# Complexity-ML/complexity-tokenizer

Hardware: AMD Instinct MI355X
Metric: MB/s raw UTF-8 encoded (encode_batch), 50k ByteLevel BPE, 1/2/4/8 MI355X (higher is better)
Workload: dtype u8

## Files before the change

complexity-tokenizer_amd/csrc/ctok_encode.cpp:

```cpp
#include <chrono>
#include <cstdio>
#include <cstring>

#include "call_plan.h"
#include "gen/unicode_data.h"
#include "host_internal.h"
#include "knobs.h"

ctok::ctok() = default;
ctok::~ctok() = default;

namespace ctok_rt __attribute__((visibility("hidden"))) {

bool cp_fast_ok() {
  static const bool ok = [] {
    if (process_knobs().no_cp_ranges) return false;
    for (uint32_t cp = 0x3000; cp < 0x1F700; cp++) {
      const int rc = cp_range_class(cp);
      if (rc < 0) continue;
      const int cl = (ct_cls_stage2[ct_cls_stage1[cp >> 8] * 64 + ((cp & 255) >> 2)] >> ((cp & 3) * 2)) & 3;
      if (cl != rc || ct_nfc_stage2[ct_nfc_stage1[cp >> 8] * 256 + (cp & 255)] != 0) return false;
    }
    return true;
  }();
// ... 331 lines not shown
  Capacities cap{};
  Work w{};
  bool tm = false;
  PassPlan plan{};
  Laps laps;
  uint64_t ntok = 0;
  uint32_t cnt[kNumCounters] = {};
};

void normalise(Enc& e, Attempt& a) {
  ctok* t = e.t;
  DeviceState* ds = e.ds;
  const EncodeCall& c = e.c;
  hipStream_t s = c.stream;
  const uint64_t n_docs = c.n_docs;
  const bool nfc = t->nfc && c.n_bytes;
  a.ev0_marker = c.timing && (t->add_prefix_space || (nfc && (c.all_nfc || !a.speculate)));
  if (a.ev0_marker) HIPTRY(hipEventRecord(ds->ev[kEvStart], s));
  ds->counters.ensure(kCounterWords);
  a.text = c.text, a.off = c.doc_off, a.B = c.n_bytes;
  a.norm = t->add_prefix_space;
  if (nfc && c.all_nfc) {
    ds->doc_flag.ensure(n_docs + 1);
    HIPTRY(hipMemsetD32Async((hipDeviceptr_t)ds->doc_flag.p, 1, n_docs + 1, s));
    a.nfc_docs = n_docs;
    a.norm = true;
  } else if (nfc && !a.speculate) {
    ds->doc_flag.ensure(n_docs + 1);
    HIPTRY(hipMemsetAsync(ds->doc_flag.p, 0, (n_docs + 1) * 4, s));
    HIPTRY(hipMemsetAsync(ds->counters.p, 0, kCounterWords * 4, s));
    a.ctr_zeroed = true;
    STEP("nfc_check", launch_nfc_check(c.text, c.n_bytes, c.doc_off, (uint32_t)n_docs, e.tb, ds->doc_flag.p,
                                       ds->counters.p + kCtrNfcDocs, s));
    HIPTRY(hipMemcpyAsync(ds->host + kPinScratch, ds->counters.p + kCtrNfcDocs, 4, hipMemcpyDeviceToHost, s));
    spin_sync(ds, s);
    a.nfc_docs = *pinned<uint32_t>(ds, kPinScratch);
    if (a.nfc_docs) a.norm = true;
  }
  if (a.norm) {
    const int do_nfc = t->nfc && a.nfc_docs;
    ds->doc_flag.ensure(n_docs + 1);
    if (!t->nfc) HIPTRY(hipMemsetAsync(ds->doc_flag.p, 0, (n_docs + 1) * 4, s));
    ds->ncp.ensure(n_docs + 1);
    ds->norm_off.ensure(n_docs + 2);
    ds->cps.ensure(4 * c.n_bytes + 64);
    STEP("norm0", launch_norm(c.text, c.doc_off, (uint32_t)n_docs, ds->doc_flag.p, t->add_prefix_space, do_nfc, e.tb,
                              ds->cps.p, ds->ncp.p, ds->norm_off.p, nullptr, 0, s));
    ds->scan_tmp.ensure(scan_tmp_elems(n_docs + 1) + 64);
    HIPTRY(scan_u64(ds->norm_off.p, n_docs, ds->scan_tmp.p, ds->scan_tmp.cap, s));
    HIPTRY(hipMemcpyAsync(ds->host + kPinScratch, ds->norm_off.p + n_docs, 8, hipMemcpyDeviceToHost, s));
    spin_sync(ds, s);
    const uint64_t nb = *pinned<uint64_t>(ds, kPinScratch);
    if (nb >= 0xF0000000ull) throw_err(CTOK_E_ARG, "normalised batch exceeds 3.75 GiB; split the batch");
    ds->norm_text.ensure(nb + 16);
    STEP("norm1", launch_norm(c.text, c.doc_off, (uint32_t)n_docs, ds->doc_flag.p, t->add_prefix_space, do_nfc, e.tb,
                              ds->cps.p, ds->ncp.p, ds->norm_off.p, ds->norm_text.p, 1, s));
    a.text = ds->norm_text.p, a.off = ds->norm_off.p, a.B = nb;
  }
  if (a.B > 0 && ((uintptr_t)a.text & 15)) throw_err(CTOK_E_ARG, "device text buffer must be 16-byte aligned");
  ds->last_norm = a.norm;
  ds->last_B = a.B;
}

template <class T, class P>
void bind(DevBuf<T>& b, size_t n, P*& field) {
  b.ensure(n);
  field = (P*)b.p;
}

void size_workspace(Enc& e, Attempt& a) {
  DeviceState* ds = e.ds;
  const ProcessKnobs& pk = process_knobs();
  Work& w = a.w;
  w.text = a.text;
  w.n_bytes = (uint32_t)a.B;
  w.doc_off = a.off;
  w.n_docs = (uint32_t)e.c.n_docs;
  w.n_words = (uint32_t)((a.B + 31) / 32);
  w.n_tiles = (uint32_t)((a.B + kTile - 1) / kTile);
  w.n_cus = ds->n_cus;
  w.nfc_watch = a.speculate ? (e.splice ? 2u : 1u) : 0u;
  w.keep_first = e.c.mode == EncodeMode::KeepFirst ? 1u : 0u;
  w.short_wgs = e.knobs.short_wgs;
  const size_t nt = w.n_tiles;
  a.cap = plan_capacities(a.B, nt, a.safe, e.tb.n_at, pk.unit, e.knobs.c3_sparse);
  w.k0 = a.cap.k0;
  w.unit = a.cap.unit;
  w.long_cap = a.cap.long_cap;
  w.mid_cap = a.cap.mid_cap;
  w.c3_max = a.cap.c3_max;
  w.rec16 = (e.t->narrow && !pk.rec32) ? 1u : 0u;
  ds->last_rec16 = (int)w.rec16;

  if (w.nfc_watch == 2) bind(ds->nfc_bits, nfc_bits_words(a.B), w.nfc_bits);
  bind(ds->tfirst, nt + 8, w.tfirst);
  bind(ds->pbits, w.n_words + 8, w.pbits);
  bind(ds->wpref, nt * 64 + 8, w.wpref);
  bind(ds->tile_np, nt + 8, w.tile_np);
  bind(ds->tile_tok, nt + 8, w.tile_tok);
  bind(ds->tile_doc, nt + 8, w.tile_doc);
  bind(ds->tcls, kNumClasses * nt + 8, w.tcls);
  bind(ds->list0, nt * w.k0 + 8, w.list0);
  bind(ds->rend, kNumClasses * nt + 8, w.rend);
  if (e.tb.n_at == 0) {
    ds->list1.ensure(nt * kCap1 + 8);
    ds->list2.ensure(nt * kCap2 + 8);
    ds->list3.ensure(nt * kCap3 + 8);
  }
  w.list1 = ds->list1.p, w.list2 = ds->list2.p, w.list3 = ds->list3.p;
  bind(ds->tcnt, nt * kTileSlots + 8, w.tcnt);
  bind(ds->prec, nt * kTileSlots * (w.rec16 ? 1 : 2) + 16, w.prec);
  bind(ds->mrec, nt * kTileSlots + 8, w.mrec);
  bind(ds->pdoc, nt * (kTileSlots / 32) + 8, w.pdoc);
  bind(ds->scratch, nt * kTileSlots + 8, w.scratch);
  bind(ds->tregion, nt + 8, w.tregion);
  bind(ds->long_list, w.long_cap + 8, w.long_list);
  bind(ds->long_cnt, w.long_cap + 8, w.long_cnt);
  bind(ds->long_ord, w.long_cap + 8, w.long_ord);
  bind(ds->long_hist, kLhWords, w.long_hist);
  bind(ds->mid_list, w.mid_cap + 8, w.mid_list);
  bind(ds->scan_tmp, std::max(scan_tmp_elems(std::max<uint64_t>(nt + 1, e.c.n_docs + 1)), tile_scan_tmp_elems(nt)) + 64,
       w.scan_tmp);
  w.scan_tmp_cap = ds->scan_tmp.cap * 2;
  w.counters = ds->counters.p;
  if (w.c3_max) {
    bind(ds->c3q, w.c3_max + 8, w.c3q);
    bind(ds->c3pre, kC3Shards + 8, w.c3pre);
  }
  w.report = (uint32_t*)(ds->host_dev + kPinReport);
  w.host_res = pk.copy_results ? nullptr : ds->host_dev + kPinNtok;
  hipStream_t s = e.c.stream;
#ifdef CTOK_CHECK
  HIPTRY(hipMemsetAsync(ds->mrec.p, 0xFF, (size_t)nt * kTileSlots * 4, s));
#endif
  if (pk.wgrec) {
    bind(ds->wgrec, kWgRecWords, w.wgrec);
    HIPTRY(hipMemsetAsync(ds->wgrec.p, 0, kWgRecWords * 8, s));
  }
  if (pk.stamps && nt) {
    bind(ds->stamps, nt * 8 + 8, w.stamps);
    HIPTRY(hipMemsetAsync(ds->stamps.p, 0, nt * 8 * 8, s));
  }
}
void bind_long_prep(DeviceState* ds, Work& w, uint32_t n_long) {
  bind(ds->long_pos, n_long + 8, w.long_pos);
  bind(ds->lw_pos, n_long + 8, w.lw_pos);
  ds->lwn.ensure(n_long + 8);
  ds->scan_tmp2.ensure(scan_tmp_elems(n_long + 1) + 64);
}
void bind_long_ids(DeviceState* ds, Work& w, uint32_t n_ids, uint32_t n_gmem_bytes) {
  bind(ds->lids, (uint64_t)n_ids + 64, w.lids);
  bind(ds->lw, 4 * (uint64_t)n_gmem_bytes + 64, w.lw);
}

Lx lx(const Enc& e, const Attempt& a, int start, int stop) {
  Lx x;
  if (a.tm && start >= 0) x.start = e.ds->ev[start];
  if (a.tm && stop >= 0) x.stop = e.ds->ev[stop];
  return x;
}


void launch_pretok(Enc& e, Attempt& a) {
  hipStream_t s = e.c.stream;
  a.tm = e.c.timing && e.c.stats && a.w.n_tiles;
  e.hp.mark(kHpPrep);
// ... 194 lines not shown
```

complexity-tokenizer_amd/csrc/ctok_internal.h:

```cpp
#pragma once
#include <hip/hip_runtime.h>

#include <cstdint>

namespace ctok_dev {

constexpr uint64_t kEmpty = ~0ull;
constexpr uint32_t kIdBits = 21;
constexpr uint64_t kKeyMask = (1ull << 42) - 1;
constexpr uint32_t kNoRank = 0x3FFFFFu;
constexpr uint32_t kMaxId = (1u << kIdBits) - 2;
constexpr uint32_t kPanicVal = kNoRank - 1;

constexpr uint32_t kErrPanic = 1u;

constexpr int kTileWords = 62;
constexpr int kTile = kTileWords * 64;
constexpr int kTileSlots = 4096;
constexpr int kSegWaves = 4;
constexpr int kSegUnroll = 4;
constexpr int kShortMax = 32;
constexpr int kMedMax = 64;
constexpr uint32_t kCap0 = kTile, kCap1 = (kTile + 8) / 9, kCap2 = (kTile + 16) / 17, kCap3 = (kTile + 32) / 33;
constexpr uint32_t kCap0Lean = 1040;
// ... 74 lines not shown
}
__host__ __device__ inline uint32_t hash16_g(uint32_t a, uint32_t b) {
  return mul24(b, 0xC2B2AFu) + mul24(a ^ 0x5A5Au, 0x27D4EBu);
}

__host__ __device__ inline uint32_t piece_hash(uint32_t lo, uint32_t hi, uint32_t len) {
  uint32_t h = mul24(lo, 0x9E3779u) + mul24((lo >> 24) | (hi << 8), 0x85EBCBu) + mul24((hi >> 16) | (len << 16), 0xC2B2AFu);
  h ^= h >> 15;
  h = mul24(h, 0x27D4EBu) ^ (h >> 9);
  return h ^ (h >> 16);
}

__host__ __device__ __forceinline__ int cp_range_class(uint32_t cp) {
  if (cp - 0x4E00u < 0x5200u) return 1;
  if (cp - 0xAC00u < 0x2BA4u) return 1;
  if (cp - 0x3041u < 0x56u) return 1;
  if (cp - 0x30A1u < 0x5Au) return 1;
  if (cp - 0x1F300u < 0x350u) return 3;
  return -1;
}

struct Tables {
  const uint64_t* merge_tab;
  uint32_t merge_mask;
  const uint4* lds_image;
  const uint32_t* pair0;
  const uint4* lds16_image;
  const uint64_t* merge16;
  uint32_t merge16_mask;
  const uint4* piece_tab;
  uint32_t piece_mask;
  const uint32_t* rank_newid;
  uint32_t n_ranks;
  const int32_t* byte2id;
  const uint8_t* cls_s1;
  const uint8_t* cls_s2;
  const uint8_t* nfc_s1;
  const uint16_t* nfc_s2;
  const uint8_t* cls_bmp;
  uint32_t cp_fast;
  const uint32_t* decomp_cp;
  const uint16_t* decomp_off;
  const uint32_t* decomp_data;
  uint32_t n_decomp;
  const uint64_t* comp_key;
  const uint32_t* comp_val;
  uint32_t n_comp;
  const uint8_t* bytemap_alnum;
  const uint8_t* at_bytes;
  const uint32_t* at_off;
  const uint32_t* at_id;
  const uint8_t* at_flags;
  uint32_t n_at;
  uint32_t proper;
  const uint32_t* eager;
  uint32_t window;
  const uint32_t* wmeta;
  uint32_t compact;
  uint32_t narrow;
  uint32_t short_packed;
  uint32_t mid_packed;
  uint32_t dbg;
  uint32_t all_bytes;
};

__host__ __device__ inline bool mid_folded(const Tables& t, uint32_t long_pieces) {
  return t.mid_packed == 2 && t.short_packed && t.n_at == 0 && long_pieces == 0;
}

struct Work {
  const uint8_t* text;
  uint32_t n_bytes;
  const uint64_t* doc_off;
  uint32_t n_docs;
  uint32_t* tfirst;
  uint32_t* pbits;
  uint32_t n_words;
  uint32_t n_tiles;
  uint32_t n_cus;
  uint32_t nfc_watch;
  uint32_t* nfc_bits;
  uint32_t mid_wide;
  uint32_t short_wgs;
  uint32_t keep_first;
  uint16_t* wpref;
  uint32_t* tile_np;
  uint32_t* tile_tok;
  uint32_t* tile_doc;
  uint32_t* tcls;
  uint32_t* list0;
  uint32_t k0;
  uint32_t* list1;
  uint32_t* list2;
  uint32_t* list3;
  void* prec;
  uint32_t rec16;
  uint32_t* mrec;
  uint32_t* pdoc;
  uint32_t* tcnt;
  uint32_t* long_cnt;
  uint32_t* long_ord;
  uint32_t* long_hist;
  uint32_t* scratch;
  uint32_t* lids;
  uint32_t* long_pos;
  uint32_t* lw_pos;
  uint32_t* rend;
  uint2* tregion;
  uint32_t long_cap, mid_cap;
  uint32_t unit;
  uint64_t* long_list;
  uint64_t* mid_list;
  uint32_t* counters;
  uint32_t* lw;
  uint32_t* scan_tmp;
  uint64_t scan_tmp_cap;
  uint64_t* stamps;
  uint32_t c3_max;
  uint32_t* c3q;
  uint32_t* c3pre;
  uint64_t* host_res;
  uint64_t* wgrec;
  uint32_t* report;
  uint32_t seq;
};

struct Lx {
  hipEvent_t start = nullptr, stop = nullptr;
};

constexpr uint32_t kDecLenMask = 0xFFFFFFu, kDecNonAscii = 1u << 30, kDecSpecial = 1u << 31;
constexpr uint32_t kDecOptSkipSpecial = 1u, kDecOptCleanup = 2u;
constexpr int kDecChunk = 4096;
constexpr int kDecTile = 4096;

struct DecTables {
  const uint2* ent;
  uint32_t n_ent;
  const uint8_t* bytes;
};

struct DecWork {
  const uint32_t* ids;
  uint32_t n_ids;
  const uint64_t* tok_off;
  uint32_t n_docs;
  uint32_t opts;
  uint32_t n_chunks;
  uint32_t* chunk_off;
  uint8_t* raw;
  uint32_t n_raw;
  uint64_t* raw_off;
  uint32_t* delbits;
  uint32_t n_tiles;
  uint32_t* tile_cnt;
  uint32_t* counters;
};

hipError_t launch_dec_len(const DecWork& w, const DecTables& t, uint32_t* tmp, uint64_t tmp_cap, hipStream_t s);
hipError_t launch_dec_gather(const DecWork& w, const DecTables& t, uint8_t* dst, uint64_t* dst_off, hipStream_t s);
hipError_t launch_dec_prepare(const DecWork& w, hipStream_t s);
hipError_t launch_dec_count(const DecWork& w, uint32_t* tmp, uint64_t tmp_cap, hipStream_t s);
hipError_t launch_dec_write(const DecWork& w, uint8_t* out, uint64_t* out_off, hipStream_t s);

constexpr uint32_t kPadItemA = 0xFFFFFFFFu;
constexpr int kPadMaxItems = 16;
// ... 79 lines not shown
```

complexity-tokenizer_amd/csrc/kernels.hip:

```cpp
#include <hip/hip_ext.h>
#include <hip/hip_runtime.h>

#include <algorithm>
#include <mutex>
#include <type_traits>

#include "ctok_internal.h"
#include "merge_packed_hd.h"
#include "seg_lane.h"

namespace ctok_dev {

#define HIPCHK(x) do { hipError_t e_ = (x); if (e_ != hipSuccess) return e_; } while (0)

template <typename F, typename... A>
static void launch_lx(const Lx& x, F k, dim3 grid, dim3 block, uint32_t lds, hipStream_t s, A... a) {
  if (x.start || x.stop)
    hipExtLaunchKernelGGL(k, grid, block, lds, s, x.start, x.stop, 0u, a...);
  else
    hipLaunchKernelGGL(k, grid, block, lds, s, a...);
}

constexpr uint32_t kNone = 0xFFFFFFFFu;
constexpr uint32_t kDead = 0xFFFFFFFFu;
constexpr uint32_t kSel = kNoRank - 1;


__device__ __forceinline__ void write_report(const Work& w) {
  const uint32_t lane = threadIdx.x & 63;
  uint32_t c3 = 0;
  if (w.c3_max) {
    const uint32_t c = w.counters[kNumCounters + lane];
    uint32_t inc = c;
#pragma unroll
    for (int o = 1; o < 64; o <<= 1) {
      const uint32_t v = (uint32_t)__shfl_up((int)inc, o, 64);
      if (lane >= (uint32_t)o) inc += v;
    }
    w.c3pre[lane] = inc - c;
    if (lane == 63) w.c3pre[64] = inc;
    c3 = __shfl((int)inc, 63, 64);
    if (__ballot(c > w.c3_max / kC3Shards)) c3 = ~0u;
  }
  if (lane < (uint32_t)kNumCounters) w.report[lane] = lane == (uint32_t)kCtrC3Count ? c3 : w.counters[lane];
  __builtin_amdgcn_fence(__ATOMIC_RELEASE, "");
  asm volatile("s_waitcnt vmcnt(0)" ::: "memory");
  if (lane == 0) __hip_atomic_store(&w.report[kNumCounters], w.seq, __ATOMIC_RELAXED, __HIP_MEMORY_SCOPE_SYSTEM);
  __builtin_amdgcn_fence(__ATOMIC_RELEASE, "");
}

__device__ __forceinline__ uint32_t wave_min_u32(uint32_t v) {
#pragma unroll
  for (int o = 32; o > 0; o >>= 1) v = min(v, (uint32_t)__shfl_xor((int)v, o, 64));
  return v;
}

__device__ __forceinline__ uint32_t wave_min_full_u32(uint32_t v) {
  v = min(v, (uint32_t)__builtin_amdgcn_update_dpp((int)v, (int)v, 0xB1, 0xF, 0xF, false));
  v = min(v, (uint32_t)__builtin_amdgcn_update_dpp((int)v, (int)v, 0x4E, 0xF, 0xF, false));
  v = min(v, (uint32_t)__builtin_amdgcn_update_dpp((int)v, (int)v, 0x141, 0xF, 0xF, false));
  v = min(v, (uint32_t)__builtin_amdgcn_update_dpp((int)v, (int)v, 0x140, 0xF, 0xF, false));
  const uint32_t a = __builtin_amdgcn_readlane(v, 0), b = __builtin_amdgcn_readlane(v, 16);
  const uint32_t c = __builtin_amdgcn_readlane(v, 32), d = __builtin_amdgcn_readlane(v, 48);
  return min(min(a, b), min(c, d));
}

__device__ __forceinline__ uint32_t wave_sum_full_u32(uint32_t v) {
  v += (uint32_t)__builtin_amdgcn_update_dpp((int)v, (int)v, 0xB1, 0xF, 0xF, false);
  v += (uint32_t)__builtin_amdgcn_update_dpp((int)v, (int)v, 0x4E, 0xF, 0xF, false);
  v += (uint32_t)__builtin_amdgcn_update_dpp((int)v, (int)v, 0x141, 0xF, 0xF, false);
  v += (uint32_t)__builtin_amdgcn_update_dpp((int)v, (int)v, 0x140, 0xF, 0xF, false);
  return __builtin_amdgcn_readlane(v, 0) + __builtin_amdgcn_readlane(v, 16) + __builtin_amdgcn_readlane(v, 32) +
         __builtin_amdgcn_readlane(v, 48);
}

__device__ __forceinline__ uint64_t lanemask_lt() {
  const uint32_t lane = threadIdx.x & 63;
  return lane ? (~0ull >> (64 - lane)) : 0ull;
}

template <typename T>
__device__ __forceinline__ T wave_incl_scan(T v) {
  const int lane = threadIdx.x & 63;
#pragma unroll
  for (int o = 1; o < 64; o <<= 1) {
    T u = __shfl_up(v, o, 64);
    if (lane >= o) v += u;
  }
  return v;
}
// ... 1090 lines not shown
    const bool has_r = q < 8;
    const uint32_t lo = lv & ((1u << bi) - 1u);
    const bool has_l = lo != 0;
    const uint32_t pv = 31u - (uint32_t)__builtin_clz(lo | 1u);
    const uint32_t L = s_tok[pv * NT + tid], R = s_tok[min(q, 7u) * NT + tid];
    s_tok[bi * NT + tid] = (uint16_t)nid;
    s_key[p * NT + tid] = ~0u;
    lv &= ~(1u << p);
    m--;
    Probe<true, HOT> pl, pr;
    pl.start(t, P, L, nid, has_l);
    pr.start(t, P, nid, R, has_r);
    const uint32_t rl = pl.finish(t, err), rr = pr.finish(t, err);
    if (has_l) s_key[pv * NT + tid] = (rl << 3) | pv;
    s_key[bi * NT + tid] = has_r ? (rr << 3) | bi : ~0u;
  }
  uint32_t* out = out_of(m);
#pragma unroll
  for (int k = 0; k < 8; k++)
    if ((lv >> k) & 1u) out[__popc(lv & ((1u << k) - 1u))] = s_tok[k * NT + tid];
  return m;
}

template <bool COMPACT, bool HOT, uint32_t NT, typename OutOf>
__device__ __forceinline__ uint32_t merge_lds8(const Tables& t, const PairLds& P, const uint32_t* tk, const uint32_t* rk,
                                               uint32_t m, lds_u32* s_key, lds_u16* s_tok, uint32_t* err,
                                               OutOf&& out_of) {
  const uint32_t tid = threadIdx.x;
#pragma unroll
  for (int k = 0; k < 8; k++) {
    s_key[k * NT + tid] = (uint32_t)k + 1 < m ? (rk[k] << 3) | (uint32_t)k : ~0u;
    s_tok[k * NT + tid] = (uint16_t)tk[k];
  }
  return merge_lds8_run<COMPACT, HOT, NT>(t, P, m, s_key, s_tok, err, out_of);
}

template <bool HOT>
struct Lookup16 {
  const Tables& t;
  const PairLds& P;
  uint32_t* err;
  Probe<true, HOT> pl, pr;
  bool has_l = false, has_r = false;
  __device__ __forceinline__ uint32_t new_id(uint32_t v) const { return v; }
  __device__ __forceinline__ void start(uint32_t L, uint32_t nid, uint32_t R, bool hl, bool hr) {
    has_l = hl;
    has_r = hr;
    pl.start(t, P, L, nid, hl);
    pr.start(t, P, nid, R, hr);
  }
  __device__ __forceinline__ void finish(uint32_t& rl, uint32_t& rr) {
    rl = (has_l ? pl.finish(t, err) : kNoRank) & 0xFFFFu;
    rr = (has_r ? pr.finish(t, err) : kNoRank) & 0xFFFFu;
  }
};

template <int K0, int K1, uint32_t NT>
__device__ __forceinline__ void lds8_store_packed(const uint32_t (&T)[8], const uint32_t (&R)[8], lds_u32* s_key,
                                                  lds_u16* s_tok) {
  if constexpr (K0 < K1) {
    s_key[K0 * NT + threadIdx.x] = mpk::lds8_key<K0>(R);
    s_tok[K0 * NT + threadIdx.x] = (uint16_t)mpk::half<K0>(T);
    lds8_store_packed<K0 + 1, K1, NT>(T, R, s_key, s_tok);
  }
}
template <int K0, int K1, int ND>
__device__ __forceinline__ void store_packed_ids(const uint32_t (&T)[ND], uint32_t m, uint32_t* out) {
  if constexpr (K0 < K1) {
    if ((uint32_t)K0 < m) out[K0] = mpk::half<K0>(T);
    store_packed_ids<K0 + 1, K1>(T, m, out);
  }
}

__device__ __forceinline__ void defer_to_generic(const Work& w, uint32_t s, uint32_t o, uint32_t n) {
  const uint32_t mi = atomicAdd(&w.counters[kCtrDropped], 1u);
  if (mi < w.mid_cap)
    w.mid_list[mi] = (uint64_t)s | ((uint64_t)o << 32) | ((uint64_t)n << 48);
  else
    atomicOr(&w.counters[kCtrOverflow], 1u);
}

template <uint32_t SORTCAP, int KT = 64>
struct PassLds {
  uint32_t pre[KT + 1], tsum[KT], tbase[KT], stat[2], bcnt[4], bfill[4], chunk, take, next;
  uint16_t perm[SORTCAP];
};

template <int N, bool COMPACT, bool HOT, uint32_t NT, uint32_t SORTCAP, bool L8 = false, int KT = 64, bool PK = false,
          bool LA = true, typename Load, int SKT>
__device__ __forceinline__ void class_pass(const Work& w, const Tables& t, const PairLds& P, const int32_t* s_b2id,
                                           PassLds<SORTCAP, SKT>& S, bool& loaded, Load&& load,
                                           lds_u32* s_key = nullptr, lds_u16* s_tok = nullptr) {
  using LC = LdsClass<N>;
  constexpr int K = KT;
  static_assert(KT <= (int)NT, "a thread per chunk tile");
  static_assert(KT <= SKT, "the shared scratch holds the pass's chunk");
  const uint32_t tid = threadIdx.x;
  uint32_t* err = &w.counters[kCtrErr];
  const uint32_t* list = class_list<N>(w);
  const uint32_t cap = class_cap<N>(w);
  const uint32_t* counts = w.tcls + (size_t)LC::cls * w.n_tiles;
  uint32_t st_bytes = 0, st_ids = 0;
  if (tid < 2) S.stat[tid] = 0;
  constexpr uint32_t blo = N == 8 ? 1 : N / 2 + 1, bw = N == 64 ? 8 : N == 32 ? 4 : 2;
  auto bucket = [&](uint32_t n) { return min(3u, (n - blo) / bw); };
  __syncthreads();
  uint32_t take = 1;
  const uint32_t U = w.unit;
  for (;;) {
    if (tid == 0) {
      S.chunk = atomicAdd(&w.counters[ctr_chunk(LC::cls)], take);
      S.take = take;
      S.next = 0;
    }
    __syncthreads();
    const uint32_t c0 = S.chunk * U;
    if (c0 >= w.n_tiles) break;
    const uint32_t tb1 = min(w.n_tiles, c0 + U * S.take);
    const uint32_t E = tile_share_init<K>(counts, tb1, c0, S.pre, S.tsum, w.tregion, LC::cls, S.tbase);
    if (E && !loaded) {
      load();
      loaded = true;
      __syncthreads();
    }
    const bool sorted = N > 8 && E <= SORTCAP;
    if (sorted) {
      if (tid < 4) { S.bcnt[tid] = 0; S.bfill[tid] = 0; }
      __syncthreads();
      for (uint32_t q = tid; q < E; q += NT) {
        const uint32_t kt = tile_of<K>(S.pre, q);
        const uint32_t b = bucket(ent_len(list[(size_t)(c0 + kt) * cap + (q - S.pre[kt])]));
#pragma unroll
        for (uint32_t bb = 0; bb < 4; bb++) {
          const uint64_t m = __ballot(b == bb);
          if (m && (threadIdx.x & 63) == __ffsll((unsigned long long)m) - 1) atomicAdd(&S.bcnt[bb], (uint32_t)__popcll(m));
        }
      }
      __syncthreads();
      if (tid == 0) {
        uint32_t acc = 0;
        for (int bb = 0; bb < 4; bb++) {
          const uint32_t c = S.bcnt[bb];
          S.bfill[bb] = acc;
          acc += c;
        }
      }
      __syncthreads();
      for (uint32_t q = tid; q < E; q += NT) {
        const uint32_t kt = tile_of<K>(S.pre, q);
        const uint32_t b = bucket(ent_len(list[(size_t)(c0 + kt) * cap + (q - S.pre[kt])]));
#pragma unroll
        for (uint32_t bb = 0; bb < 4; bb++) {
          const uint32_t slot = wave_append(&S.bfill[bb], b == bb);
          if (b == bb) S.perm[slot] = (uint16_t)q;
        }
      }
      __syncthreads();
    }
    auto entry = [&](uint32_t i, uint32_t& kt) {
      const uint32_t q = sorted ? (uint32_t)S.perm[i] : i;
      kt = tile_of<K>(S.pre, q);
      return list[(size_t)(c0 + kt) * cap + (q - S.pre[kt])];
    };
    auto start_of = [&](uint32_t e, uint32_t kt) { return (c0 + kt) * kTile + (e & 0xFFFu); };
    auto body = [&](uint32_t e, uint32_t kt, const uint32_t* wv, auto&& hook) {
        const uint32_t tile = c0 + kt;
        const uint32_t s = tile * kTile + (e & 0xFFFu);
        const uint32_t o = ent_ord(e);
        const uint32_t n = ent_len(e);
        uint32_t pos = 0;
        auto out_of = [&](uint32_t mm) {
          pos = atomicAdd(&S.tsum[kt], mm);
          return w.scratch + (size_t)tile * kTileSlots + pos;
        };
        auto record = [&](uint32_t m) {
          CTOK_CHECK_REC(m >= 1 && m <= n && pos + m <= (uint32_t)kTileSlots && o < (uint32_t)kTileSlots,
                         "[ctok check] class pass N=%d PK=%d tile %u: record m=%u n=%u pos=%u ordinal=%u\n", N, (int)PK,
                         tile, m, n, pos, o);
          w.mrec[(size_t)tile * kTileSlots + o] = rec_short(m, pos);
          st_bytes += n;
          st_ids += m;
        };
        if constexpr (PK) {
          static_assert((N == 16 || N == 32) && L8 && COMPACT,
                        "the packed tiers are the 9..16 B and 17..32 B passes', ahead of merge_lds8, on compact tables");
          constexpr int ND = N / 2;
          uint32_t T[ND], R[ND], bytes[N];
          bool missing = false;
#pragma unroll
          for (int k = 0; k < N; k++) bytes[k] = byte_of(wv[k >> 2], k);
#pragma unroll
          for (int d = 0; d < ND; d++) {
            const int32_t i0 = s_b2id[bytes[2 * d]], i1 = s_b2id[bytes[2 * d + 1]];
            missing |= (((uint32_t)(2 * d) < n) & (i0 < 0)) | (((uint32_t)(2 * d + 1) < n) & (i1 < 0));
            T[d] = mpk::pack2((uint32_t)i0, (uint32_t)i1);
          }
          if (missing) {
            hook();
            defer_to_generic(w, s, o, n);
            return;
          }
          {
            uint32_t v[N];
#pragma unroll
            for (int k = 0; k < N - 1; k++) v[k] = t.pair0[(bytes[k] << 8) | bytes[k + 1]];
            v[N - 1] = kNoRank;
#pragma unroll
            for (int k = 0; k < N - 1; k++) v[k] = (uint32_t)k + 1 < n ? v[k] : kNoRank;
#pragma unroll
            for (int d = 0; d < ND; d++) R[d] = mpk::pack2(v[2 * d], v[2 * d + 1]);
          }
          uint32_t m = n;
          Lookup16<HOT> lk{t, P, err};
          if constexpr (N == 32) {
            bool more = mpk::tier(T, R, m, 16u, lk);
            uint32_t T8[8], R8[8];
            mpk::low_half(T, T8);
            mpk::low_half(R, R8);
            if (more) more = mpk::tier(T8, R8, m, 8u, lk);
            hook();
            if (more) {
              lds8_store_packed<0, 8, NT>(T8, R8, s_key, s_tok);
              m = merge_lds8_run<COMPACT, HOT, NT>(t, P, m, s_key, s_tok, err, out_of);
            } else if (m > 16) {
              store_packed_ids<0, N>(T, m, out_of(m));
            } else {
              store_packed_ids<0, 16>(T8, m, out_of(m));
            }
          } else {
            const bool more = mpk::tier(T, R, m, 8u, lk);
            hook();
            if (more) {
              lds8_store_packed<0, 8, NT>(T, R, s_key, s_tok);
              m = merge_lds8_run<COMPACT, HOT, NT>(t, P, m, s_key, s_tok, err, out_of);
            } else {
              store_packed_ids<0, N>(T, m, out_of(m));
            }
          }
          record(m);
          return;
        }
        uint32_t tk[N], rk[N];
        bool missing = false;
// ... 2365 lines not shown
```

complexity-tokenizer_amd/csrc/knobs.h:

```cpp
#pragma once
#include <cstdint>
#include <cstdlib>
#include <optional>

#include "ctok_internal.h"

namespace ctok_rt __attribute__((visibility("hidden"))) {

inline bool env_set(const char* name) { return getenv(name) != nullptr; }
inline int env_int(const char* name, int dflt) {
  const char* v = getenv(name);
  return v ? atoi(v) : dflt;
}
inline std::optional<uint64_t> env_u64(const char* name) {
  const char* v = getenv(name);
  return v ? std::optional<uint64_t>(strtoull(v, nullptr, 10)) : std::nullopt;
}

struct LoadKnobs {
  bool load_timing = env_set("CTOK_LOAD_TIMING");
  bool force_wide = env_set("CTOK_FORCE_WIDE");
  bool no_hot_table = env_set("CTOK_NO_HOT_TABLE");
  bool no_window = env_set("CTOK_NO_WINDOW");
  bool no_piece_table = env_set("CTOK_NO_PIECE_TABLE");
  size_t merge_slack = (size_t)env_int("CTOK_MERGE_SLACK", 8);
  size_t merge16_slack = (size_t)env_int("CTOK_MERGE16_SLACK", 64);
  size_t piece_slack = (size_t)env_int("CTOK_PIECE_SLACK", 8);
};

struct UploadKnobs {
  bool force_improper = env_set("CTOK_FORCE_IMPROPER");
  bool force_wide_slots = env_set("CTOK_FORCE_WIDE_SLOTS");
  int short_packed = env_int("CTOK_SHORT_PACKED", 1);
  int mid_packed = env_int("CTOK_MID_PACKED", ctok_dev::kMidPackedDefault);
  uint32_t dbg_mode = (uint32_t)env_int("CTOK_DBG_MODE", 0);
};

struct ProcessKnobs {
  bool no_cp_ranges = env_set("CTOK_NO_CP_RANGES");
  bool debug_sync = env_set("CTOK_DEBUG_SYNC");
  bool safe_capacities = env_set("CTOK_SAFE_CAPACITIES");
  bool hostprof = env_set("CTOK_HOSTPROF");
  uint32_t unit = (uint32_t)env_int("CTOK_UNIT", 0);
  bool rec32 = env_set("CTOK_REC32");
  bool wgrec = env_set("CTOK_WGREC");
  bool stamps = env_set("CTOK_STAMPS");
  bool copy_results = env_set("CTOK_COPY_RESULTS");
  bool no_chunk_ramp = env_set("CTOK_NO_CHUNK_RAMP");
  bool pipe_trace = env_set("CTOK_PIPE_TRACE");
};
inline const ProcessKnobs& process_knobs() {
  static const ProcessKnobs k;
  return k;
}

struct CallKnobs {
  bool no_nfc_speculation = env_set("CTOK_NO_NFC_SPECULATION");
  bool nfc_rerun = env_set("CTOK_NFC_RERUN");
  uint32_t short_wgs = (uint32_t)env_int("CTOK_SHORT_WGS", 0);
  std::optional<uint64_t> c3_sparse = env_u64("CTOK_C3_SPARSE");
  bool mid512 = env_set("CTOK_MID512");
  int overlap = env_int("CTOK_OVERLAP", ctok_dev::kOverlapDefault);
  bool wire32 = env_set("CTOK_WIRE32");
};

}
```

Baseline: 172,700.

## Sort chunk entries by exact piece length with single-pass atomic bucket ranking

Measured after the change: 176,900, median of 6. +2.5%, better.

```diff
diff --git a/complexity-tokenizer_amd/csrc/chunk_sort_hd.h b/complexity-tokenizer_amd/csrc/chunk_sort_hd.h
--- /dev/null
+++ b/complexity-tokenizer_amd/csrc/chunk_sort_hd.h
@@ -0,0 +1,39 @@
+#pragma once
+#include <cstdint>
+
+#if defined(__HIPCC__)
+#define CSORT_HD __host__ __device__ __forceinline__
+#else
+#define CSORT_HD inline
+#endif
+
+namespace csort {
+
+constexpr uint32_t kMaxBuckets = 16;
+
+constexpr uint32_t kExact8 = 1u, kExact16 = 2u, kExact32 = 4u, kAscending = 8u;
+constexpr uint32_t kModeMask = 15u;
+constexpr uint32_t kModeDefault = kExact16 | kExact32;
+
+CSORT_HD constexpr uint32_t exact_bit(int N) { return N == 8 ? kExact8 : N == 16 ? kExact16 : N == 32 ? kExact32 : 0u; }
+CSORT_HD constexpr bool sorts(int N, uint32_t mode) { return N != 8 || (mode & kExact8) != 0; }
+CSORT_HD constexpr bool exact(int N, uint32_t mode) { return (mode & exact_bit(N)) != 0; }
+
+CSORT_HD constexpr uint32_t class_lo(int N) { return N == 8 ? 1u : (uint32_t)N / 2 + 1; }
+CSORT_HD constexpr uint32_t coarse_shift(int N) { return N == 64 ? 3u : N == 32 ? 2u : 1u; }
+
+CSORT_HD constexpr uint32_t n_buckets(int N, bool ex) { return !ex ? 4u : N == 16 ? 8u : N == 32 ? 16u : 4u; }
+
+CSORT_HD uint32_t bucket(int N, bool ex, uint32_t n) {
+  const uint32_t lo = ex && N == 8 ? 5u : class_lo(N), nb = n_buckets(N, ex);
+  const uint32_t b = (n < lo ? 0u : n - lo) >> (ex ? 0u : coarse_shift(N));
+  return b < nb ? b : nb - 1u;
+}
+
+CSORT_HD uint32_t code(int N, uint32_t mode, uint32_t n) {
+  const bool ex = exact(N, mode);
+  const uint32_t b = bucket(N, ex, n);
+  return (mode & kAscending) ? b : n_buckets(N, ex) - 1u - b;
+}
+
+}
diff --git a/complexity-tokenizer_amd/csrc/ctok_encode.cpp b/complexity-tokenizer_amd/csrc/ctok_encode.cpp
--- a/complexity-tokenizer_amd/csrc/ctok_encode.cpp
+++ b/complexity-tokenizer_amd/csrc/ctok_encode.cpp
@@ -437,6 +437,7 @@
   w.nfc_watch = a.speculate ? (e.splice ? 2u : 1u) : 0u;
   w.keep_first = e.c.mode == EncodeMode::KeepFirst ? 1u : 0u;
   w.short_wgs = e.knobs.short_wgs;
+  w.chunk_sort = e.knobs.chunk_sort;
   const size_t nt = w.n_tiles;
   a.cap = plan_capacities(a.B, nt, a.safe, e.tb.n_at, pk.unit, e.knobs.c3_sparse);
   w.k0 = a.cap.k0;
diff --git a/complexity-tokenizer_amd/csrc/ctok_internal.h b/complexity-tokenizer_amd/csrc/ctok_internal.h
--- a/complexity-tokenizer_amd/csrc/ctok_internal.h
+++ b/complexity-tokenizer_amd/csrc/ctok_internal.h
@@ -180,6 +180,7 @@
   uint32_t* nfc_bits;
   uint32_t mid_wide;
   uint32_t short_wgs;
+  uint32_t chunk_sort;
   uint32_t keep_first;
   uint16_t* wpref;
   uint32_t* tile_np;
diff --git a/complexity-tokenizer_amd/csrc/kernels.hip b/complexity-tokenizer_amd/csrc/kernels.hip
--- a/complexity-tokenizer_amd/csrc/kernels.hip
+++ b/complexity-tokenizer_amd/csrc/kernels.hip
@@ -6,6 +6,7 @@
 #include <type_traits>
 
 #include "ctok_internal.h"
+#include "chunk_sort_hd.h"
 #include "merge_packed_hd.h"
 #include "seg_lane.h"
 
@@ -1262,9 +1263,53 @@
 
 template <uint32_t SORTCAP, int KT = 64>
 struct PassLds {
-  uint32_t pre[KT + 1], tsum[KT], tbase[KT], stat[2], bcnt[4], bfill[4], chunk, take, next;
+  uint32_t pre[KT + 1], tsum[KT], tbase[KT], stat[2], bcnt[csort::kMaxBuckets], bfill[csort::kMaxBuckets], chunk, take, next;
   uint16_t perm[SORTCAP];
 };
+
+template <int N, int K, uint32_t NT, uint32_t SORTCAP, class PL>
+__device__ __forceinline__ void chunk_sort(PL& S, const uint32_t* list, uint32_t c0, uint32_t cap, uint32_t Es,
+                                           uint32_t mode) {
+  static_assert(SORTCAP <= 65536, "perm holds u16 entry numbers, a rank fits 16 bits");
+  constexpr uint32_t G = 4, EPT = (SORTCAP + G * NT - 1) / (G * NT) * G;
+  uint32_t tid = threadIdx.x;
+  asm volatile("" : "+v"(tid));
+  uint32_t cr[EPT];
+#pragma unroll
+  for (uint32_t j = 0; j < EPT; j++) cr[j] = 0;
+#pragma unroll
+  for (uint32_t g = 0; g < EPT; g += G) {
+    if (g * NT < Es) {
+      uint32_t e[G];
+#pragma unroll
+      for (uint32_t j = 0; j < G; j++) {
+        const uint32_t q = min(tid + (g + j) * NT, Es - 1);
+        const uint32_t kt = tile_of<K>(S.pre, q);
+        e[j] = list[(size_t)(c0 + kt) * cap + (q - S.pre[kt])];
+      }
+#pragma unroll
+      for (uint32_t j = 0; j < G; j++) {
+        if (tid + (g + j) * NT < Es) {
+          const uint32_t c = csort::code(N, mode, ent_len(e[j]));
+          cr[g + j] = (c << 16) | atomicAdd(&S.bcnt[c], 1u);
+        }
+      }
+    }
+  }
+  __syncthreads();
+  if (tid < 64) {
+    const uint32_t c = tid < csort::kMaxBuckets ? S.bcnt[tid] : 0u;
+    const uint32_t inc = wave_incl_scan(c);
+    if (tid < csort::kMaxBuckets) S.bfill[tid] = inc - c;
+  }
+  __syncthreads();
+#pragma unroll
+  for (uint32_t j = 0; j < EPT; j++) {
+    const uint32_t q = tid + j * NT;
+    if (q < Es) S.perm[S.bfill[cr[j] >> 16] + (cr[j] & 0xFFFFu)] = (uint16_t)q;
+  }
+  __syncthreads();
+}
 
 template <int N, bool COMPACT, bool HOT, uint32_t NT, uint32_t SORTCAP, bool L8 = false, int KT = 64, bool PK = false,
           bool LA = true, typename Load, int SKT>
@@ -1282,8 +1327,7 @@
   const uint32_t* counts = w.tcls + (size_t)LC::cls * w.n_tiles;
   uint32_t st_bytes = 0, st_ids = 0;
   if (tid < 2) S.stat[tid] = 0;
-  constexpr uint32_t blo = N == 8 ? 1 : N / 2 + 1, bw = N == 64 ? 8 : N == 32 ? 4 : 2;
-  auto bucket = [&](uint32_t n) { return min(3u, (n - blo) / bw); };
+  const uint32_t mode = w.chunk_sort;
   __syncthreads();
   uint32_t take = 1;
   const uint32_t U = w.unit;
@@ -1293,6 +1337,7 @@
       S.take = take;
       S.next = 0;
     }
+    if (tid < csort::kMaxBuckets) S.bcnt[tid] = 0;
     __syncthreads();
     const uint32_t c0 = S.chunk * U;
     if (c0 >= w.n_tiles) break;
@@ -1303,42 +1348,49 @@
       loaded = true;
       __syncthreads();
     }
-    const bool sorted = N > 8 && E <= SORTCAP;
-    if (sorted) {
-      if (tid < 4) { S.bcnt[tid] = 0; S.bfill[tid] = 0; }
-      __syncthreads();
-      for (uint32_t q = tid; q < E; q += NT) {
-        const uint32_t kt = tile_of<K>(S.pre, q);
-        const uint32_t b = bucket(ent_len(list[(size_t)(c0 + kt) * cap + (q - S.pre[kt])]));
-#pragma unroll
-        for (uint32_t bb = 0; bb < 4; bb++) {
-          const uint64_t m = __ballot(b == bb);
-          if (m && (threadIdx.x & 63) == __ffsll((unsigned long long)m) - 1) atomicAdd(&S.bcnt[bb], (uint32_t)__popcll(m));
-        }
-      }
-      __syncthreads();
-      if (tid == 0) {
-        uint32_t acc = 0;
-        for (int bb = 0; bb < 4; bb++) {
-          const uint32_t c = S.bcnt[bb];
-          S.bfill[bb] = acc;
-          acc += c;
-        }
-      }
-      __syncthreads();
-      for (uint32_t q = tid; q < E; q += NT) {
-        const uint32_t kt = tile_of<K>(S.pre, q);
-        const uint32_t b = bucket(ent_len(list[(size_t)(c0 + kt) * cap + (q - S.pre[kt])]));
-#pragma unroll
-        for (uint32_t bb = 0; bb < 4; bb++) {
-          const uint32_t slot = wave_append(&S.bfill[bb], b == bb);
-          if (b == bb) S.perm[slot] = (uint16_t)q;
-        }
-      }
-      __syncthreads();
+    uint32_t Es = 0;
+    if constexpr (N > 32) {
+      if (E <= SORTCAP) {
+        Es = uni(E);
+        auto bucket = [&](uint32_t n) { return csort::bucket(N, false, n); };
+        if (tid < 4) { S.bcnt[tid] = 0; S.bfill[tid] = 0; }
+        __syncthreads();
+        for (uint32_t q = tid; q < E; q += NT) {
+          const uint32_t kt = tile_of<K>(S.pre, q);
+          const uint32_t b = bucket(ent_len(list[(size_t)(c0 + kt) * cap + (q - S.pre[kt])]));
+#pragma unroll
+          for (uint32_t bb = 0; bb < 4; bb++) {
+            const uint64_t m = __ballot(b == bb);
+            if (m && (threadIdx.x & 63) == __ffsll((unsigned long long)m) - 1) atomicAdd(&S.bcnt[bb], (uint32_t)__popcll(m));
+          }
+        }
+        __syncthreads();
+        if (tid == 0) {
+          uint32_t acc = 0;
+          for (int bb = 0; bb < 4; bb++) {
+            const uint32_t c = S.bcnt[bb];
+            S.bfill[bb] = acc;
+            acc += c;
+          }
+        }
+        __syncthreads();
+        for (uint32_t q = tid; q < E; q += NT) {
+          const uint32_t kt = tile_of<K>(S.pre, q);
+          const uint32_t b = bucket(ent_len(list[(size_t)(c0 + kt) * cap + (q - S.pre[kt])]));
+#pragma unroll
+          for (uint32_t bb = 0; bb < 4; bb++) {
+            const uint32_t slot = wave_append(&S.bfill[bb], b == bb);
+            if (b == bb) S.perm[slot] = (uint16_t)q;
+          }
+        }
+        __syncthreads();
+      }
+    } else if (csort::sorts(N, mode)) {
+      Es = uni(min(E, SORTCAP));
+      chunk_sort<N, K, NT, SORTCAP>(S, list, c0, cap, Es, mode);
     }
     auto entry = [&](uint32_t i, uint32_t& kt) {
-      const uint32_t q = sorted ? (uint32_t)S.perm[i] : i;
+      const uint32_t q = i < Es ? (uint32_t)S.perm[i] : i;
       kt = tile_of<K>(S.pre, q);
       return list[(size_t)(c0 + kt) * cap + (q - S.pre[kt])];
     };
diff --git a/complexity-tokenizer_amd/csrc/knobs.h b/complexity-tokenizer_amd/csrc/knobs.h
--- a/complexity-tokenizer_amd/csrc/knobs.h
+++ b/complexity-tokenizer_amd/csrc/knobs.h
@@ -4,6 +4,7 @@
 #include <optional>
 
 #include "ctok_internal.h"
+#include "chunk_sort_hd.h"
 
 namespace ctok_rt __attribute__((visibility("hidden"))) {
 
@@ -58,6 +59,7 @@
   bool no_nfc_speculation = env_set("CTOK_NO_NFC_SPECULATION");
   bool nfc_rerun = env_set("CTOK_NFC_RERUN");
   uint32_t short_wgs = (uint32_t)env_int("CTOK_SHORT_WGS", 0);
+  uint32_t chunk_sort = (uint32_t)env_int("CTOK_CHUNK_SORT", (int)csort::kModeDefault) & csort::kModeMask;
   std::optional<uint64_t> c3_sparse = env_u64("CTOK_C3_SPARSE");
   bool mid512 = env_set("CTOK_MID512");
   int overlap = env_int("CTOK_OVERLAP", ctok_dev::kOverlapDefault);
```
